# Skylarking/MARL

Hardware: AMD Instinct MI355X
Metric: env_steps_per_sec (higher is better)
Workload: dtype f32 (bf16x6 split products, fp32 accumulate)

## Files before the change

marl_amd/csrc/common.h:

```cpp
#pragma once
#include <hip/hip_runtime.h>
#include <stdint.h>

#define MARL_WAVE 64

#define WG_BARRIER() asm volatile("s_waitcnt lgkmcnt(0)\n\ts_barrier" ::: "memory")

struct MarlSwitches {
  int fwd_xs, fwd_w2l, bwd_pipe_max_rt, wgrad_tall, wide_res, rollout_v1, unroll_r6;
};
extern "C" const MarlSwitches* marl_switches(void);

#ifndef MARL_PAD_H
#define MARL_PAD_H 8
#endif
#ifndef MARL_PAD_K
#define MARL_PAD_K 8
#endif
#ifndef MARL_PAD_G
#define MARL_PAD_G 8
#endif

typedef float f32x4 __attribute__((ext_vector_type(4)));
typedef int i32x4 __attribute__((ext_vector_type(4)));

__device__ __forceinline__ f32x4 mfma16(float a, float b, f32x4 c) {
  return __builtin_amdgcn_mfma_f32_16x16x4f32(a, b, c, 0, 0, 0);
}

__device__ __forceinline__ f32x4 mfma16x4(const f32x4& a, const f32x4& b, f32x4 c) {
  c = mfma16(a[0], b[0], c);
  c = mfma16(a[1], b[1], c);
  c = mfma16(a[2], b[2], c);
  c = mfma16(a[3], b[3], c);
  return c;
}

#ifdef MARL_NO_INTERLEAVE
__device__ __forceinline__ void mfma16x4_il2(const f32x4& a0, const f32x4& b0, f32x4& c0, const f32x4& a1, const f32x4& b1, f32x4& c1) {
  c0 = mfma16x4(a0, b0, c0); c1 = mfma16x4(a1, b1, c1);
}
__device__ __forceinline__ void mfma16x4_il3(const f32x4& a0, const f32x4& b0, f32x4& c0, const f32x4& a1, const f32x4& b1, f32x4& c1,
// ... 250 lines not shown
```

marl_amd/csrc/optim.hip:

```cpp
#include "common.h"
#include <string.h>
#include "../../include/marl_hip.h"

namespace {
constexpr int TPB = 256;
constexpr int MAXB = 1024;

__global__ void sumsq_kernel(const float* g, long n, float* ws) {
  __shared__ float sh[TPB / 64];
  float s = 0.f;
  for (long i = (long)blockIdx.x * TPB + threadIdx.x; i < n; i += (long)gridDim.x * TPB) s += g[i] * g[i];
  s = wave_sum(s);
  if ((threadIdx.x & 63) == 0) sh[threadIdx.x >> 6] = s;
  __syncthreads();
  if (threadIdx.x == 0) ws[blockIdx.x] = sh[0] + sh[1] + sh[2] + sh[3];
}

__global__ void sumsq_finish_kernel(const float* ws, int nb, float* out) {
  __shared__ float sh[TPB];
  float s = 0.f;
  for (int b = threadIdx.x; b < nb; b += TPB) s += ws[b];
  sh[threadIdx.x] = s;
  __syncthreads();
  for (int o = TPB / 2; o > 0; o >>= 1) {
// ... 42 lines not shown
}
}

extern "C" size_t marl_sumsq_workspace(long n) { return MAXB * sizeof(float); }

extern "C" int marl_grad_sumsq(const float* g, long n, float* sumsq, float* ws, void* stream) {
  const int nb = blocks_for(n);
  hipLaunchKernelGGL(sumsq_kernel, dim3(nb), dim3(TPB), 0, (hipStream_t)stream, g, n, ws);
  MARL_CHECK_LAUNCH();
  hipLaunchKernelGGL(sumsq_finish_kernel, dim3(1), dim3(TPB), 0, (hipStream_t)stream, (const float*)ws, nb, sumsq);
  MARL_CHECK_LAUNCH();
  return 0;
}

extern "C" int marl_rmsprop_step(float* p, const float* g, float* sq, long n, float lr, float alpha, float eps,
                                 float clip, const float* sumsq, const float* den, void* stream) {
  if (n <= 0) return 0;
  hipLaunchKernelGGL(rmsprop_kernel, dim3(blocks_for(n)), dim3(TPB), 0, (hipStream_t)stream, p, g, sq, n, lr, alpha,
                     eps, clip, sumsq, den);
  MARL_CHECK_LAUNCH();
  return 0;
}

extern "C" int marl_adam_step(float* p, const float* g, float* m, float* v, long n, float lr, float beta1,
                              float beta2, float eps, float bc1, float bc2_sqrt, float clip, const float* sumsq,
                              const float* den, void* stream) {
  if (n <= 0) return 0;
  hipLaunchKernelGGL(adam_kernel, dim3(blocks_for(n)), dim3(TPB), 0, (hipStream_t)stream, p, g, m, v, n, lr, beta1,
                     beta2, eps, bc1, bc2_sqrt, clip, sumsq, den);
  MARL_CHECK_LAUNCH();
  return 0;
}

static MarlSwitches g_switches = {1, 1, 4, 1, 1, 0, 1};
extern "C" const MarlSwitches* marl_switches(void) { return &g_switches; }
static int* switch_slot(const char* name) {
  if (!name) return nullptr;
  struct { const char* n; int* p; } tab[] = {{"fwd_xs", &g_switches.fwd_xs}, {"fwd_w2l", &g_switches.fwd_w2l},
                                             {"bwd_pipe_max_rt", &g_switches.bwd_pipe_max_rt}, {"wgrad_tall", &g_switches.wgrad_tall},
                                             {"wide_res", &g_switches.wide_res}, {"rollout_v1", &g_switches.rollout_v1}, {"unroll_r6", &g_switches.unroll_r6}};
  for (auto& t : tab)
    if (!strcmp(t.n, name)) return t.p;
  return nullptr;
}
extern "C" int marl_experiment_set(const char* name, int value) {
  int* p = switch_slot(name);
  if (!p) return -1;
  *p = value;
  return 0;
}
extern "C" int marl_experiment_get(const char* name) {
  int* p = switch_slot(name);
  return p ? *p : (-2147483647 - 1);
}

#ifndef MARL_SRC_HASH
#define MARL_SRC_HASH "unknown"
#endif
extern "C" const char* marl_hip_version(void) { return "marl_hip 0.4 (gfx950) src " MARL_SRC_HASH; }
```

marl_amd/csrc/qmix_fused.hip:

```cpp
#include "x6.h"
#include "../../include/marl_hip.h"

namespace {

constexpr int E = 32;
constexpr int KCQ = 8;
constexpr int SS = 128 + 4;
constexpr int NAG = 5;
constexpr int PP = 136;

struct QmixArgs {
  const float *W[4], *Bv[4];
  const float *wb2, *bb2;
  ConcatSrc s;
  const float* q;
  const float* g;
  float* q_tot;
  float* dq;
  float* ws;
  const float *lr, *lterm, *lpadded, *lq_tgt;
  float gamma;
  long rows;
  int N, S, C;
};

__host__ __device__ inline long qmix_slab_floats(int C, int S) { return (long)C * (S + 1) + (E + 1) + 2; }

template <int CTRL>
__device__ __forceinline__ float dpp(float v) {
  return __builtin_bit_cast(float, __builtin_amdgcn_update_dpp(0, __builtin_bit_cast(int, v), CTRL, 0xf, 0xf, true));
}
constexpr int DPP_XOR1 = 0xB1, DPP_XOR2 = 0x4E;
constexpr int DPP_HALF_MIRROR = 0x141, DPP_MIRROR = 0x140;
constexpr int DPP_ROR4 = 0x124, DPP_ROR8 = 0x128;
template <int EW>
__device__ __forceinline__ float group_sum(float v) {
  if (EW == 4) v += dpp<DPP_ROR4>(v);
  v += dpp<DPP_ROR8>(v);
  return v;
}
template <int EW>
__device__ __forceinline__ float e_sum(float v) {
  v += dpp<DPP_XOR1>(v);
  v += dpp<DPP_XOR2>(v);
  if (EW == 8) v += dpp<DPP_HALF_MIRROR>(v);
  return v;
}
__device__ __forceinline__ float row_sum(float v) {
  v += dpp<DPP_XOR1>(v);
  v += dpp<DPP_XOR2>(v);
  v += dpp<DPP_HALF_MIRROR>(v);
  v += dpp<DPP_MIRROR>(v);
  return v;
}
__device__ __forceinline__ float sign_clamp(float x, float lo) { return __builtin_amdgcn_fmed3f(x * 0x1p126f, lo, 1.0f); }

template <bool BWD, int NW, bool LOSS = false, bool X6 = false>
__global__ __launch_bounds__(64 * NW, 2) void qmix_fused_kernel(QmixArgs a) {
  static_assert(!LOSS || BWD, "the loss is folded into the backward kernel");
  static_assert(!X6 || NW == 8, "the split variant runs eight waves (two column tiles per wave: 96 registers of pre-split weights)");
  constexpr int QNT = 64 * NW, EW = 32 / NW, GPT = 16 / EW, TPW = 8 / GPT, LT = TPW - 1;
  constexpr int SRAW = X6 ? 2 * 3 * 16 * PP * 2 : 2 * 16 * SS * 4;
  __shared__ __attribute__((aligned(16))) char Sraw[SRAW];
  float (*Ss)[16 * SS] = reinterpret_cast<float (*)[16 * SS]>(Sraw);
  short* const Sp = reinterpret_cast<short*>(Sraw);
  constexpr int PLN = 16 * PP, PBUF = 3 * PLN;
  constexpr int KR = (X6 && BWD) ? (LOSS ? 2 : 3) : 4;
  constexpr int KL = 4 - KR;
  __shared__ __attribute__((aligned(16))) i32x4 WL[KL ? NW * TPW * KL * 3 * 64 : 1];
  __shared__ __attribute__((aligned(16))) float Qt2[2][8][16];
  __shared__ __attribute__((aligned(16))) float QT[NW][16];
  __shared__ __attribute__((aligned(16))) float DQP[NW][NAG][16];
  __shared__ __attribute__((aligned(16))) float Gs2[2][16];
  __shared__ __attribute__((aligned(16))) float Ls2[2][4][16];
  const int tid = threadIdx.x, lane = tid & 63, wave = tid >> 6;
  const int q4 = lane >> 4, m = lane & 15;
  const int el = m & (EW - 1), gl = m / EW, e = EW * wave + el;
  const int N = a.N, S = a.S, C = a.C, NE = N * E;
  const bool ones = S < 128;

  f32x4 wq[X6 ? 1 : TPW][X6 ? 1 : KCQ];
  F3 wq6[X6 ? TPW : 1][X6 ? KR : 1];
  float bias[TPW];
  int grp[TPW];
#pragma unroll
  for (int c = 0; c < TPW; ++c) {
    const int g = GPT * c + gl;
    grp[c] = g;
    const float *Wp = nullptr, *Bp = nullptr;
    if (g < NAG) { if (g < N) { Wp = a.W[0] + (long)(g * E + e) * S; Bp = a.Bv[0] + g * E + e; } }
    else { Wp = a.W[g - NAG + 1] + (long)e * S; Bp = a.Bv[g - NAG + 1] + e; }
    bias[c] = Bp ? *Bp : 0.f;
    if (X6) {
#pragma unroll
      for (int kc = 0; kc < 4; ++kc) {
        float v[8];
#pragma unroll
        for (int jj = 0; jj < 8; ++jj) {
          const int kk = 32 * kc + 8 * q4 + jj;
          v[jj] = (Wp && kk < S) ? Wp[kk] : 0.f;
        }
        const F3 f = split8((f32x4){v[0], v[1], v[2], v[3]}, (f32x4){v[4], v[5], v[6], v[7]});
        if (kc < KR) wq6[c][kc < KR ? kc : 0] = f;
        else { i32x4* wl = WL + (((wave * TPW + c) * (KL ? KL : 1) + (kc - KR)) * 3) * 64 + lane; wl[0] = f.h; wl[64] = f.m; wl[128] = f.l; }
      }
    } else {
#pragma unroll
      for (int kc = 0; kc < KCQ; ++kc)
#pragma unroll
        for (int i = 0; i < 4; ++i) {
          const int kk = 16 * kc + 4 * q4 + i;
          wq[c][kc][i] = (Wp && kk < S) ? Wp[kk] : 0.f;
        }
    }
  }
  const bool is6 = grp[LT] == 6, is7 = grp[LT] == 7;
  const float wb2e = a.wb2[e];
  const float cw = is7 ? wb2e : 0.f;
  const float bb2 = a.bb2[0];
  constexpr int MT = NAG / GPT;
  const unsigned absmask = grp[MT] < NAG ? 0x7fffffffu : 0xffffffffu;
  float lo_c[TPW];
#pragma unroll
  for (int c = 0; c < TPW; ++c) lo_c[c] = grp[c] == NAG ? 1.f : (grp[c] == 7 ? 0.f : -1.f);

  f32x4 accW[BWD ? TPW : 1][BWD ? KCQ : 1];
  float sbW[TPW];
#pragma unroll
  for (int c = 0; c < TPW; ++c) sbW[c] = 0.f;
  float acc_wb2 = 0.f, acc_bb2 = 0.f;
  float acc_ln = 0.f, acc_lm = 0.f;
  if (BWD) {
#pragma unroll
    for (int c = 0; c < TPW; ++c)
#pragma unroll
      for (int kc = 0; kc < KCQ; ++kc) accW[c][kc] = (f32x4){0.f, 0.f, 0.f, 0.f};
  }
  if (tid < 2 * 8 * 16) {
    const int r8 = (tid >> 4) & 7;
    (&Qt2[0][0][0])[tid] = r8 == NAG ? 1.f : 0.f;
  }

  const int tiles = (int)((a.rows + 15) / 16);
  constexpr int NPF = 512 / QNT;
  f32x4 pf[NPF];
  int pe0 = 0, pe1 = 0, pw0 = 0, pw1 = 0;
  const int fr = tid >> 5, fc4 = (tid & 31) * 4;
  const bool ones_lane = BWD && ones && fc4 == (S & ~3);
  const int ones_j = S & 3;
  const int nrows = (int)a.rows;
  const unsigned last_row = (unsigned)(nrows - 1);
  const unsigned rpe = (unsigned)a.s.rpe0;
  const int roff = rpe ? (int)a.s.off0 : 0;
  const FastDiv fd = a.s.fd0;
  const int* emap = a.s.emap0;
  const float* sp0 = a.s.p0 + (fc4 < S ? fc4 : 0);
  const long ld = a.s.ld0, blk = (long)a.s.bs0 * a.s.ld0;
  auto map_one = [&](int tile, int i, int& pe, int& pw) {
    unsigned row = (unsigned)tile * 16u + (unsigned)(fr + (QNT / 32) * i);
    row = row < last_row ? row : last_row;
    const unsigned ep = rpe ? fastdiv(row, fd) : 0u;
    pw = (int)(row - ep * rpe) + roff;
    pe = (int)ep;
    if (emap) pe = emap[ep];
  };
  auto map_issue = [&](int tile) {
    map_one(tile, 0, pe0, pw0);
    if (NPF > 1) map_one(tile, 1, pe1, pw1);
  };
  auto fetch_one = [&](int pe, int pw) {
    f32x4 v = *reinterpret_cast<const f32x4*>(sp0 + ((long)pe * blk + (long)pw * ld));
    if (BWD) {
#pragma unroll
      for (int j = 0; j < 4; ++j) v[j] = (ones_lane && j == ones_j) ? 1.f : v[j];
    }
    return v;
  };
  auto fetch = [&](int) {
    pf[0] = fetch_one(pe0, pw0);
    if (NPF > 1) pf[NPF - 1] = fetch_one(pe1, pw1);
  };
  auto stash = [&](int buf) {
#pragma unroll
    for (int i = 0; i < NPF; ++i) {
      if (X6) {
        const F3h f = split4(pf[i]);
        short* p = Sp + buf * PBUF + (fr + (QNT / 32) * i) * PP + fc4;
        *reinterpret_cast<i32x2*>(p) = f.h;
        *reinterpret_cast<i32x2*>(p + PLN) = f.m;
        *reinterpret_cast<i32x2*>(p + 2 * PLN) = f.l;
      } else *reinterpret_cast<f32x4*>(&Ss[buf][(fr + (QNT / 32) * i) * SS + fc4]) = pf[i];
    }
  };
  float pq = 0.f, pg = 0.f, pl[4] = {0.f, 0.f, 0.f, 0.f};
  const int qr = tid / N, qn = tid - qr * N;
  auto fetch_qg = [&](int tile) {
    pq = 0.f; pg = 0.f;
    if (tid < 16 * N) {
      const int row = tile * 16 + qr;
      if (row < nrows) pq = a.q[(unsigned)(row * N + qn)];
    }
    if (BWD && tid >= 192 && tid < 208) {
      const int row = tile * 16 + (tid - 192);
      if (LOSS) {
        pl[0] = pl[1] = pl[3] = 0.f; pl[2] = 1.f;
        if (row < nrows) { pl[0] = a.lr[row]; pl[1] = a.lterm[row]; pl[2] = a.lpadded[row]; pl[3] = a.lq_tgt[row]; }
      } else if (row < nrows) pg = a.g[row];
    }
  };
  auto flush_dq = [&](int prow0) {
    if (tid < 16 * N) {
      float v = 0.f;
#pragma unroll
      for (int w = 0; w < NW; ++w) v += DQP[w][qn][qr];
      if (prow0 + qr < nrows) a.dq[(unsigned)((prow0 + qr) * N + qn)] = v;
    }
  };
  int tile = blockIdx.x;
  if (tile < tiles) {
    map_issue(tile); fetch(tile); fetch_qg(tile);
    if (tile + (int)gridDim.x < tiles) map_issue(tile + gridDim.x);
    stash(0);
  }
  int buf = 0;
  int prow0 = -1;
  ST_DECL(8);
  __syncthreads();
  for (; tile < tiles; tile += gridDim.x, buf ^= 1) {
    const int row0 = tile * 16;
    if (tid < 16 * N) Qt2[buf][qn][qr] = pq;
    if (BWD && tid >= 192 && tid < 208) {
      if (LOSS) {
#pragma unroll
        for (int k = 0; k < 4; ++k) Ls2[buf][k][tid - 192] = pl[k];
      } else Gs2[buf][tid - 192] = pg;
    }
    const int nt = tile + gridDim.x;
    if (nt < tiles) {
      fetch(nt); fetch_qg(nt);
      if (nt + (int)gridDim.x < tiles) map_issue(nt + gridDim.x);
    }
    ST_MARK(0);
    WG_BARRIER();
    ST_MARK(1);
    if (BWD && prow0 >= 0) flush_dq(prow0);
    f32x4 acc[TPW];
#pragma unroll
    for (int c = 0; c < TPW; ++c) acc[c] = (f32x4){bias[c], bias[c], bias[c], bias[c]};
    if (X6) {
      f32x4 accb[TPW];
#pragma unroll
      for (int c = 0; c < TPW; ++c) accb[c] = (f32x4){0.f, 0.f, 0.f, 0.f};
      const short* sp = Sp + buf * PBUF + m * PP + 8 * q4;
#pragma unroll
      for (int kc = 0; kc < 4; ++kc) {
        F3 xa;
        xa.h = *reinterpret_cast<const i32x4*>(sp + 32 * kc);
        xa.m = *reinterpret_cast<const i32x4*>(sp + PLN + 32 * kc);
        xa.l = *reinterpret_cast<const i32x4*>(sp + 2 * PLN + 32 * kc);
        F3 wk[TPW];
#pragma unroll
        for (int c = 0; c < TPW; ++c) {
          if (kc < KR) wk[c] = wq6[c][kc < KR ? kc : 0];
          else { const i32x4* wl = WL + (((wave * TPW + c) * (KL ? KL : 1) + (kc - KR)) * 3) * 64 + lane; wk[c].h = wl[0]; wk[c].m = wl[64]; wk[c].l = wl[128]; }
        }
#define OP(p_, q_) _Pragma("unroll") for (int c = 0; c < TPW; ++c) { if (kc & 1) accb[c] = mm(xa.p_, wk[c].q_, accb[c]); else acc[c] = mm(xa.p_, wk[c].q_, acc[c]); }
        OP(m, m) OP(h, l) OP(l, h) OP(h, m) OP(m, h) OP(h, h)
#undef OP
      }
#pragma unroll
      for (int c = 0; c < TPW; ++c) acc[c] += accb[c];
    } else {
      const float* sr = &Ss[buf][m * SS + 4 * q4];
#pragma unroll
      for (int kc = 0; kc < KCQ; ++kc) {
        const f32x4 a4 = *reinterpret_cast<const f32x4*>(sr + 16 * kc);
#pragma unroll
        for (int i = 0; i < 4; ++i)
#pragma unroll
          for (int c = 0; c < TPW; ++c) acc[c] = mfma16(a4[i], wq[c][kc][i], acc[c]);
      }
    }
    ST_MARK(2);
    __builtin_amdgcn_sched_barrier(0);
    f32x4 qv[TPW];
    f32x4 p = {0.f, 0.f, 0.f, 0.f};
#pragma unroll
    for (int c = 0; c <= MT; ++c) {
      qv[c] = *reinterpret_cast<const f32x4*>(&Qt2[buf][grp[c]][4 * q4]);
#pragma unroll
      for (int i = 0; i < 4; ++i) {
        const float av = acc[c][i];
        const float x = c < MT ? fabsf(av) : __builtin_bit_cast(float, __builtin_bit_cast(unsigned, av) & absmask);
        p[i] = c == 0 ? x * qv[c][i] : fmaf(x, qv[c][i], p[i]);
      }
    }
    f32x4 ex, hid, t4;
#pragma unroll
    for (int i = 0; i < 4; ++i) {
      p[i] = group_sum<EW>(p[i]);
      ex[i] = __expf(p[i]);
      hid[i] = p[i] > 0.f ? p[i] : ex[i] - 1.f;
      const float z = is6 ? fabsf(acc[LT][i]) : fmaxf(acc[LT][i], 0.f);
      t4[i] = row_sum(z * (is6 ? hid[i] : cw));
    }
    if (m == 0) *reinterpret_cast<f32x4*>(&QT[wave][4 * q4]) = t4;
    ST_MARK(3);
    WG_BARRIER();
    ST_MARK(4);
    if (!BWD) {
      if (tid < 16) {
        float tot = 0.f;
#pragma unroll
        for (int w = 0; w < NW; ++w) tot += QT[w][tid];
        if (row0 + tid < nrows) a.q_tot[row0 + tid] = tot + bb2;
      }
      ST_MARK(5);
    } else {
      f32x4 qt = *reinterpret_cast<const f32x4*>(&QT[0][4 * q4]);
#pragma unroll
      for (int w = 1; w < NW; ++w) qt += *reinterpret_cast<const f32x4*>(&QT[w][4 * q4]);
      f32x4 gr;
      if (LOSS) {
        const f32x4 lr = *reinterpret_cast<const f32x4*>(&Ls2[buf][0][4 * q4]);
        const f32x4 lt = *reinterpret_cast<const f32x4*>(&Ls2[buf][1][4 * q4]);
        const f32x4 lp = *reinterpret_cast<const f32x4*>(&Ls2[buf][2][4 * q4]);
        const f32x4 lq = *reinterpret_cast<const f32x4*>(&Ls2[buf][3][4 * q4]);
#pragma unroll
        for (int i = 0; i < 4; ++i) {
          qt[i] += bb2;
          const float mask = 1.f - lp[i];
          const float target = lr[i] + a.gamma * lq[i] * (1.f - lt[i]);
          const float mtd = mask * (target - qt[i]);
          gr[i] = -2.f * mask * mtd;
          acc_ln += mtd * mtd; acc_lm += mask;
        }
        if (a.q_tot && wave == 0 && m == 0) {
          if (row0 + 16 <= nrows) *reinterpret_cast<f32x4*>(&a.q_tot[row0 + 4 * q4]) = qt;
          else {
#pragma unroll
            for (int i = 0; i < 4; ++i) if (row0 + 4 * q4 + i < nrows) a.q_tot[row0 + 4 * q4 + i] = qt[i];
          }
        }
      } else gr = *reinterpret_cast<const f32x4*>(&Gs2[buf][4 * q4]);
      f32x4 dpre, dhy[TPW];
#pragma unroll
      for (int i = 0; i < 4; ++i) {
        const float w2 = group_sum<EW>(is6 ? fabsf(acc[LT][i]) : 0.f);
        dpre[i] = gr[i] * w2 * (p[i] > 0.f ? 1.f : ex[i]);
        acc_wb2 += gr[i] * fmaxf(acc[LT][i], 0.f);
        acc_bb2 += gr[i];
      }
#pragma unroll
      for (int c = 0; c < TPW; ++c) {
        const bool lo_all = GPT * c + GPT - 1 <= NAG, hi_all = GPT * c > NAG;
#pragma unroll
        for (int i = 0; i < 4; ++i) {
          float x, y;
          if (lo_all) { x = qv[c][i]; y = dpre[i]; }
          else if (hi_all) { x = gr[i]; y = is6 ? hid[i] : wb2e; }
          else {
            const bool lo = grp[c] <= NAG;
            x = lo ? qv[c][i] : gr[i];
            y = lo ? dpre[i] : (is6 ? hid[i] : wb2e);
          }
          dhy[c][i] = (x * y) * sign_clamp(acc[c][i], lo_c[c]);
        }
        if (!ones) sbW[c] += dhy[c][0] + dhy[c][1] + dhy[c][2] + dhy[c][3];
        if (GPT * c < NAG) {
          f32x4 d4;
#pragma unroll
          for (int i = 0; i < 4; ++i) d4[i] = e_sum<EW>(fabsf(acc[c][i]) * dpre[i]);
          if (el == 0 && grp[c] < N) *reinterpret_cast<f32x4*>(&DQP[wave][grp[c]][4 * q4]) = d4;
        }
      }
      ST_MARK(5);
      __builtin_amdgcn_sched_barrier(0);
      if (X6) {
        typedef __attribute__((address_space(3))) s16x4 lds_s16x4;
        F3h dA[TPW];
#pragma unroll
        for (int c = 0; c < TPW; ++c) dA[c] = split4(dhy[c]);
        const short* tb = Sp + buf * PBUF + (4 * q4 + (m >> 2)) * PP + 4 * (m & 3);
#pragma unroll
        for (int kc = 0; kc < KCQ; ++kc) {
          F3h sb;
          sb.h = __builtin_bit_cast(i32x2, __builtin_amdgcn_ds_read_tr16_b64_v4i16((lds_s16x4*)(tb + 16 * kc)));
          sb.m = __builtin_bit_cast(i32x2, __builtin_amdgcn_ds_read_tr16_b64_v4i16((lds_s16x4*)(tb + PLN + 16 * kc)));
          sb.l = __builtin_bit_cast(i32x2, __builtin_amdgcn_ds_read_tr16_b64_v4i16((lds_s16x4*)(tb + 2 * PLN + 16 * kc)));
#define OP(p_, q_) _Pragma("unroll") for (int c = 0; c < TPW; ++c) accW[c][kc] = mmh(dA[c].p_, sb.q_, accW[c][kc]);
          OP(m, m) OP(h, l) OP(l, h) OP(h, m) OP(m, h) OP(h, h)
#undef OP
        }
      } else {
        const float* sd = &Ss[buf][(4 * q4) * SS + m];
#pragma unroll
        for (int kc = 0; kc < KCQ; ++kc) {
          f32x4 sD;
#pragma unroll
          for (int i = 0; i < 4; ++i) sD[i] = sd[i * SS + 16 * kc];
#pragma unroll
          for (int i = 0; i < 4; ++i)
#pragma unroll
            for (int c = 0; c < TPW; ++c) accW[c][kc] = mfma16(dhy[c][i], sD[i], accW[c][kc]);
        }
      }
      prow0 = row0;
    }
    ST_MARK(6);
    if (nt < tiles) stash(buf ^ 1);
    ST_MARK(7);
  }
  ST_DUMP_AT(8, BWD ? 8 : 0);
  if (BWD) {
    __syncthreads();
    if (prow0 >= 0) flush_dq(prow0);
    float* slab = a.ws + (long)blockIdx.x * qmix_slab_floats(C, S);
    const int Sx = S + 1;
#pragma unroll
    for (int c = 0; c < TPW; ++c) {
#pragma unroll
      for (int i = 0; i < 4; ++i) {
        const int cc = 4 * q4 + i, g = GPT * c + cc / EW, ee = EW * wave + (cc & (EW - 1));
        if (g < NAG && g >= N) continue;
        const int col = g < NAG ? g * E + ee : NE + (g - NAG) * E + ee;
#pragma unroll
        for (int kc = 0; kc < KCQ; ++kc) {
          const int k = 16 * kc + m;
          if (k < S || (ones && k == S)) slab[(long)col * Sx + k] = accW[c][kc][i];
        }
      }
      if (!ones) {
        float sb = sbW[c];
        sb += __shfl_xor(sb, 16, 64); sb += __shfl_xor(sb, 32, 64);
        const int g = grp[c];
        if (q4 == 0 && !(g < NAG && g >= N)) slab[(long)(g < NAG ? g * E + e : NE + (g - NAG) * E + e) * Sx + S] = sb;
      }
    }
    float v = acc_wb2;
    v += __shfl_xor(v, 16, 64); v += __shfl_xor(v, 32, 64);
    if (is7 && q4 == 0) slab[(long)C * Sx + e] = v;
    float b = acc_bb2, ln = acc_ln, lm = acc_lm;
    b += __shfl_xor(b, 16, 64); b += __shfl_xor(b, 32, 64);
    ln += __shfl_xor(ln, 16, 64); ln += __shfl_xor(ln, 32, 64);
    lm += __shfl_xor(lm, 16, 64); lm += __shfl_xor(lm, 32, 64);
    if (tid == 0) {
      slab[(long)C * Sx + E] = b;
      slab[(long)C * Sx + E + 1] = LOSS ? ln : 0.f;
      slab[(long)C * Sx + E + 2] = LOSS ? lm : 0.f;
    }
  }
// ... 71 lines not shown

}

extern "C" int marl_qmix_fused_supported(int N, int S, int Eq) { return supported(N, S, Eq) ? 1 : 0; }

extern "C" size_t marl_qmix_fused_workspace(long rows, int N, int S) {
  return (size_t)grid_for(rows) * qmix_slab_floats(N * E + 3 * E, S) * sizeof(float);
}

static int qmix_fwd_impl(const marl_qmix_weights_t* w, const marl_src_t* s, const float* q, float* q_tot,
                         long rows, int N, int S, int Eq, bool x6, void* stream) {
  if (rows <= 0) return 0;
  if (!supported(N, S, Eq)) return (int)hipErrorInvalidValue;
  QmixArgs a;
  if (fill(a, w, s, q, rows, N, S)) return (int)hipErrorInvalidValue;
  a.g = nullptr; a.q_tot = q_tot; a.dq = nullptr; a.ws = nullptr;
  a.lr = a.lterm = a.lpadded = a.lq_tgt = nullptr; a.gamma = 0.f;
  if (x6) hipLaunchKernelGGL((qmix_fused_kernel<false, 8, false, true>), dim3(grid_for(rows, 1)), dim3(512), 0, (hipStream_t)stream, a);
  else hipLaunchKernelGGL((qmix_fused_kernel<false, 4>), dim3(grid_for(rows, 2)), dim3(256), 0, (hipStream_t)stream, a);
  MARL_CHECK_LAUNCH();
  return 0;
}
extern "C" int marl_qmix_fused_fwd(const marl_qmix_weights_t* w, const marl_src_t* s, const float* q, float* q_tot,
                                   long rows, int N, int S, int Eq, void* stream) {
  return qmix_fwd_impl(w, s, q, q_tot, rows, N, S, Eq, false, stream);
}
extern "C" int marl_qmix_fused_fwd_x6(const marl_qmix_weights_t* w, const marl_src_t* s, const float* q, float* q_tot,
                                      long rows, int N, int S, int Eq, void* stream) {
  return qmix_fwd_impl(w, s, q, q_tot, rows, N, S, Eq, true, stream);
}

static int qmix_bwd_launch(QmixArgs& a, const marl_qmix_weights_t* grads, float* loss2, float* ws, long rows, int N, int S,
                           bool loss, bool x6, hipStream_t st) {
  const unsigned nwg = grid_for(rows);
  if (x6) {
    if (loss) hipLaunchKernelGGL((qmix_fused_kernel<true, 8, true, true>), dim3(nwg), dim3(512), 0, st, a);
    else hipLaunchKernelGGL((qmix_fused_kernel<true, 8, false, true>), dim3(nwg), dim3(512), 0, st, a);
  } else if (loss) hipLaunchKernelGGL((qmix_fused_kernel<true, 8, true>), dim3(nwg), dim3(512), 0, st, a);
  else hipLaunchKernelGGL((qmix_fused_kernel<true, 8, false>), dim3(nwg), dim3(512), 0, st, a);
  MARL_CHECK_LAUNCH();
  QmixRedArgs r;
  r.ws = ws; r.nwg = (int)nwg; r.N = N; r.S = S; r.C = a.C; r.loss2 = loss2;
  r.dW[0] = const_cast<float*>(grads->w1); r.dB[0] = const_cast<float*>(grads->w1_b);
  r.dW[1] = const_cast<float*>(grads->b1); r.dB[1] = const_cast<float*>(grads->b1_b);
  r.dW[2] = const_cast<float*>(grads->w2); r.dB[2] = const_cast<float*>(grads->w2_b);
  r.dW[3] = const_cast<float*>(grads->h); r.dB[3] = const_cast<float*>(grads->h_b);
  r.dwb2 = const_cast<float*>(grads->b2_w); r.dbb2 = const_cast<float*>(grads->b2_b);
  const long slab = qmix_slab_floats(a.C, S);
  hipLaunchKernelGGL(qmix_fused_reduce_kernel, dim3((unsigned)((slab + 63) / 64)), dim3(64 * RSG), 0, st, r);
  MARL_CHECK_LAUNCH();
  return 0;
}

static int qmix_bwd_impl(const marl_qmix_weights_t* w, const marl_src_t* s, const float* q, const float* dq_tot, float* dq,
                         const marl_qmix_weights_t* grads, float* ws, size_t ws_bytes, long rows, int N, int S, int Eq, bool x6,
                         void* stream) {
  if (rows <= 0) return 0;
  if (!supported(N, S, Eq)) return (int)hipErrorInvalidValue;
  if (ws_bytes < marl_qmix_fused_workspace(rows, N, S)) return (int)hipErrorInvalidValue;
  QmixArgs a;
  if (fill(a, w, s, q, rows, N, S)) return (int)hipErrorInvalidValue;
  a.g = dq_tot; a.q_tot = nullptr; a.dq = dq; a.ws = ws;
  a.lr = a.lterm = a.lpadded = a.lq_tgt = nullptr; a.gamma = 0.f;
  return qmix_bwd_launch(a, grads, nullptr, ws, rows, N, S, false, x6, (hipStream_t)stream);
}
extern "C" int marl_qmix_fused_bwd(const marl_qmix_weights_t* w, const marl_src_t* s, const float* q,
                                   const float* dq_tot, float* dq, const marl_qmix_weights_t* grads, float* ws,
                                   size_t ws_bytes, long rows, int N, int S, int Eq, void* stream) {
// ... 38 lines not shown
```

marl_amd/experiments.py:

```python
from __future__ import annotations

import contextlib
import os
import warnings

LIB_DEFAULTS = {"fwd_xs": 1, "fwd_w2l": 1, "bwd_pipe_max_rt": 4, "wgrad_tall": 1, "wide_res": 1, "rollout_v1": 0, "unroll_r6": 1}
HOST_DEFAULTS = {"no_pair": 0, "no_chain": 0, "chain_split": None, "mlp3_keep": 1, "x6_bwd_min_wg": 1, "force_reducer": 0}


def _env_int(name, default):
    v = os.environ.get("MARL_" + name.upper())
    if v is None or v == "":
        return default
    try:
        return int(v)
    except ValueError:
        warnings.warn("MARL_%s=%r ignored (want an integer)" % (name.upper(), v))
        return default


_lib_values = {k: _env_int(k, d) for k, d in LIB_DEFAULTS.items()}
_host_values = {k: _env_int(k, d) for k, d in HOST_DEFAULTS.items()}
if _host_values["chain_split"] is not None and not (_host_values["chain_split"] == 0 or
                                                      (8 <= _host_values["chain_split"] <= 248 and _host_values["chain_split"] % 8 == 0)):
    warnings.warn("MARL_CHAIN_SPLIT=%r ignored (want 0 or a multiple of 8 in 8..248)" % _host_values["chain_split"])
    _host_values["chain_split"] = None
_applied = None
generation = 0


def apply(lib):
    global _applied
    _applied = lib
    for k, v in _lib_values.items():
        if v != LIB_DEFAULTS[k]:
            rc = lib.marl_experiment_set(k.encode(), int(v))
            assert rc == 0, "marl_experiment_set(%s) failed" % k


# ... 35 lines not shown
```

Measured before the change: 72.23 million.

## Process row-tile pairs in split QMIX backward to double weight-gradient MFMA K

Adds a PAIR variant of the split-precision QMIX backward kernel in which each iteration handles two 16-row tiles. The weight-gradient MFMAs then consume 32 rows of K via paired transposed LDS reads and split8. Prefetch moves after the elementwise stage, and fewer weight k-chunks stay in registers. It is enabled by default when there are at least 512 tiles, and the grid is halved and capped at 256. The aim is fewer MFMA issues per row and less loop overhead, at the cost of doubled LDS staging, more register pressure and spilling weight chunks to LDS.

```diff
diff --git a/marl_amd/csrc/common.h b/marl_amd/csrc/common.h
--- a/marl_amd/csrc/common.h
+++ b/marl_amd/csrc/common.h
@@ -7,7 +7,7 @@
 #define WG_BARRIER() asm volatile("s_waitcnt lgkmcnt(0)\n\ts_barrier" ::: "memory")
 
 struct MarlSwitches {
-  int fwd_xs, fwd_w2l, bwd_pipe_max_rt, wgrad_tall, wide_res, rollout_v1, unroll_r6;
+  int fwd_xs, fwd_w2l, bwd_pipe_max_rt, wgrad_tall, wide_res, rollout_v1, unroll_r6, qmix_pair;
 };
 extern "C" const MarlSwitches* marl_switches(void);
 
diff --git a/marl_amd/csrc/optim.hip b/marl_amd/csrc/optim.hip
--- a/marl_amd/csrc/optim.hip
+++ b/marl_amd/csrc/optim.hip
@@ -98,13 +98,14 @@
   return 0;
 }
 
-static MarlSwitches g_switches = {1, 1, 4, 1, 1, 0, 1};
+static MarlSwitches g_switches = {1, 1, 4, 1, 1, 0, 1, 0};
 extern "C" const MarlSwitches* marl_switches(void) { return &g_switches; }
 static int* switch_slot(const char* name) {
   if (!name) return nullptr;
   struct { const char* n; int* p; } tab[] = {{"fwd_xs", &g_switches.fwd_xs}, {"fwd_w2l", &g_switches.fwd_w2l},
                                              {"bwd_pipe_max_rt", &g_switches.bwd_pipe_max_rt}, {"wgrad_tall", &g_switches.wgrad_tall},
-                                             {"wide_res", &g_switches.wide_res}, {"rollout_v1", &g_switches.rollout_v1}, {"unroll_r6", &g_switches.unroll_r6}};
+                                             {"wide_res", &g_switches.wide_res}, {"rollout_v1", &g_switches.rollout_v1}, {"unroll_r6", &g_switches.unroll_r6},
+                                             {"qmix_pair", &g_switches.qmix_pair}};
   for (auto& t : tab)
     if (!strcmp(t.n, name)) return t.p;
   return nullptr;
diff --git a/marl_amd/csrc/qmix_fused.hip b/marl_amd/csrc/qmix_fused.hip
--- a/marl_amd/csrc/qmix_fused.hip
+++ b/marl_amd/csrc/qmix_fused.hip
@@ -55,24 +55,26 @@
 }
 __device__ __forceinline__ float sign_clamp(float x, float lo) { return __builtin_amdgcn_fmed3f(x * 0x1p126f, lo, 1.0f); }
 
-template <bool BWD, int NW, bool LOSS = false, bool X6 = false>
+template <bool BWD, int NW, bool LOSS = false, bool X6 = false, bool PAIR = false>
 __global__ __launch_bounds__(64 * NW, 2) void qmix_fused_kernel(QmixArgs a) {
   static_assert(!LOSS || BWD, "the loss is folded into the backward kernel");
   static_assert(!X6 || NW == 8, "the split variant runs eight waves (two column tiles per wave: 96 registers of pre-split weights)");
+  static_assert(!PAIR || (BWD && X6), "row-tile pairs exist for the weight gradient of the split backward kernels");
   constexpr int QNT = 64 * NW, EW = 32 / NW, GPT = 16 / EW, TPW = 8 / GPT, LT = TPW - 1;
-  constexpr int SRAW = X6 ? 2 * 3 * 16 * PP * 2 : 2 * 16 * SS * 4;
+  constexpr int NTP = PAIR ? 2 : 1;
+  constexpr int SRAW = X6 ? 2 * NTP * 3 * 16 * PP * 2 : 2 * 16 * SS * 4;
   __shared__ __attribute__((aligned(16))) char Sraw[SRAW];
   float (*Ss)[16 * SS] = reinterpret_cast<float (*)[16 * SS]>(Sraw);
   short* const Sp = reinterpret_cast<short*>(Sraw);
-  constexpr int PLN = 16 * PP, PBUF = 3 * PLN;
-  constexpr int KR = (X6 && BWD) ? (LOSS ? 2 : 3) : 4;
+  constexpr int PLN = 16 * PP, PTL = 3 * PLN, PBUF = NTP * PTL;
+  constexpr int KR = (X6 && BWD) ? ((LOSS || PAIR) ? 2 : 3) : 4;
   constexpr int KL = 4 - KR;
   __shared__ __attribute__((aligned(16))) i32x4 WL[KL ? NW * TPW * KL * 3 * 64 : 1];
-  __shared__ __attribute__((aligned(16))) float Qt2[2][8][16];
-  __shared__ __attribute__((aligned(16))) float QT[NW][16];
-  __shared__ __attribute__((aligned(16))) float DQP[NW][NAG][16];
-  __shared__ __attribute__((aligned(16))) float Gs2[2][16];
-  __shared__ __attribute__((aligned(16))) float Ls2[2][4][16];
+  __shared__ __attribute__((aligned(16))) float Qt2[2][NTP][8][16];
+  __shared__ __attribute__((aligned(16))) float QT[NTP][NW][16];
+  __shared__ __attribute__((aligned(16))) float DQP[NTP][NW][NAG][16];
+  __shared__ __attribute__((aligned(16))) float Gs2[2][NTP][16];
+  __shared__ __attribute__((aligned(16))) float Ls2[2][NTP][4][16];
   const int tid = threadIdx.x, lane = tid & 63, wave = tid >> 6;
   const int q4 = lane >> 4, m = lane & 15;
   const int el = m & (EW - 1), gl = m / EW, e = EW * wave + el;
@@ -136,17 +138,33 @@
 #pragma unroll
       for (int kc = 0; kc < KCQ; ++kc) accW[c][kc] = (f32x4){0.f, 0.f, 0.f, 0.f};
   }
-  if (tid < 2 * 8 * 16) {
+  if (tid < 2 * NTP * 8 * 16) {
     const int r8 = (tid >> 4) & 7;
-    (&Qt2[0][0][0])[tid] = r8 == NAG ? 1.f : 0.f;
+    (&Qt2[0][0][0][0])[tid] = r8 == NAG ? 1.f : 0.f;
   }
 
-  const int tiles = (int)((a.rows + 15) / 16);
-  constexpr int NPF = 512 / QNT;
+  const int tiles = (int)((a.rows + 16 * NTP - 1) / (16 * NTP));
+  constexpr int NPF = NTP * 512 / QNT;
   f32x4 pf[NPF];
   int pe0 = 0, pe1 = 0, pw0 = 0, pw1 = 0;
-  const int fr = tid >> 5, fc4 = (tid & 31) * 4;
-  const bool ones_lane = BWD && ones && fc4 == (S & ~3);
+  struct Ix { int fr, fc4, qr, qn, qj, qi, gj, gi; bool ones_lane; const float* sp0; };
+  auto mk_ix = [&](int t) {
+    Ix x;
+    x.fr = t >> 5; x.fc4 = (t & 31) * 4;
+    x.ones_lane = BWD && ones && x.fc4 == (S & ~3);
+    x.sp0 = a.s.p0 + (x.fc4 < S ? x.fc4 : 0);
+    x.qr = t / N; x.qn = t - x.qr * N;
+    x.qj = PAIR ? x.qr >> 4 : 0; x.qi = PAIR ? x.qr & 15 : x.qr;
+    x.gj = PAIR ? (t - 192) >> 4 : 0; x.gi = PAIR ? (t - 192) & 15 : t - 192;
+    return x;
+  };
+  const Ix ix0 = mk_ix(tid);
+  auto ix = [&]() {
+    if (!PAIR) return ix0;
+    int t = tid;
+    asm volatile("" : "+v"(t));
+    return mk_ix(t);
+  };
   const int ones_j = S & 3;
   const int nrows = (int)a.rows;
   const unsigned last_row = (unsigned)(nrows - 1);
@@ -154,10 +172,9 @@
   const int roff = rpe ? (int)a.s.off0 : 0;
   const FastDiv fd = a.s.fd0;
   const int* emap = a.s.emap0;
-  const float* sp0 = a.s.p0 + (fc4 < S ? fc4 : 0);
   const long ld = a.s.ld0, blk = (long)a.s.bs0 * a.s.ld0;
   auto map_one = [&](int tile, int i, int& pe, int& pw) {
-    unsigned row = (unsigned)tile * 16u + (unsigned)(fr + (QNT / 32) * i);
+    unsigned row = (unsigned)tile * (16u * NTP) + (unsigned)(ix().fr + (QNT / 32) * i);
     row = row < last_row ? row : last_row;
     const unsigned ep = rpe ? fastdiv(row, fd) : 0u;
     pw = (int)(row - ep * rpe) + roff;
@@ -169,10 +186,11 @@
     if (NPF > 1) map_one(tile, 1, pe1, pw1);
   };
   auto fetch_one = [&](int pe, int pw) {
-    f32x4 v = *reinterpret_cast<const f32x4*>(sp0 + ((long)pe * blk + (long)pw * ld));
+    const Ix x = ix();
+    f32x4 v = *reinterpret_cast<const f32x4*>(x.sp0 + ((long)pe * blk + (long)pw * ld));
     if (BWD) {
 #pragma unroll
-      for (int j = 0; j < 4; ++j) v[j] = (ones_lane && j == ones_j) ? 1.f : v[j];
+      for (int j = 0; j < 4; ++j) v[j] = (x.ones_lane && j == ones_j) ? 1.f : v[j];
     }
     return v;
   };
@@ -181,11 +199,12 @@
     if (NPF > 1) pf[NPF - 1] = fetch_one(pe1, pw1);
   };
   auto stash = [&](int buf) {
+    const int fr = ix().fr, fc4 = ix().fc4;
 #pragma unroll
     for (int i = 0; i < NPF; ++i) {
       if (X6) {
         const F3h f = split4(pf[i]);
-        short* p = Sp + buf * PBUF + (fr + (QNT / 32) * i) * PP + fc4;
+        short* p = Sp + buf * PBUF + (PAIR ? i * PTL + fr * PP : (fr + (QNT / 32) * i) * PP) + fc4;
         *reinterpret_cast<i32x2*>(p) = f.h;
         *reinterpret_cast<i32x2*>(p + PLN) = f.m;
         *reinterpret_cast<i32x2*>(p + 2 * PLN) = f.l;
@@ -193,15 +212,24 @@
     }
   };
   float pq = 0.f, pg = 0.f, pl[4] = {0.f, 0.f, 0.f, 0.f};
-  const int qr = tid / N, qn = tid - qr * N;
   auto fetch_qg = [&](int tile) {
     pq = 0.f; pg = 0.f;
-    if (tid < 16 * N) {
-      const int row = tile * 16 + qr;
-      if (row < nrows) pq = a.q[(unsigned)(row * N + qn)];
-    }
-    if (BWD && tid >= 192 && tid < 208) {
-      const int row = tile * 16 + (tid - 192);
+    if (tid < 16 * NTP * N) {
+      const Ix x = ix();
+      const int row = tile * (16 * NTP) + x.qr;
+      if (row < nrows) pq = a.q[(unsigned)(row * N + x.qn)];
+    }
+    if (PAIR && LOSS) {
+      if (tid >= 192 && tid < 320) {
+        int t = tid - 192;
+        asm volatile("" : "+v"(t));
+        const int k = t >> 5, row = tile * 32 + (t & 31);
+        pg = k == 2 ? 1.f : 0.f;
+        const float* src = k == 0 ? a.lr : (k == 1 ? a.lterm : (k == 2 ? a.lpadded : a.lq_tgt));
+        if (row < nrows) pg = src[row];
+      }
+    } else if (BWD && tid >= 192 && tid < 192 + 16 * NTP) {
+      const int row = tile * (16 * NTP) + (tid - 192);
       if (LOSS) {
         pl[0] = pl[1] = pl[3] = 0.f; pl[2] = 1.f;
         if (row < nrows) { pl[0] = a.lr[row]; pl[1] = a.lterm[row]; pl[2] = a.lpadded[row]; pl[3] = a.lq_tgt[row]; }
@@ -209,11 +237,12 @@
     }
   };
   auto flush_dq = [&](int prow0) {
-    if (tid < 16 * N) {
+    if (tid < 16 * NTP * N) {
+      const Ix x = ix();
       float v = 0.f;
 #pragma unroll
-      for (int w = 0; w < NW; ++w) v += DQP[w][qn][qr];
-      if (prow0 + qr < nrows) a.dq[(unsigned)((prow0 + qr) * N + qn)] = v;
+      for (int w = 0; w < NW; ++w) v += DQP[x.qj][w][x.qn][x.qi];
+      if (prow0 + x.qr < nrows) a.dq[(unsigned)((prow0 + x.qr) * N + x.qn)] = v;
     }
   };
   int tile = blockIdx.x;
@@ -227,49 +256,71 @@
   ST_DECL(8);
   __syncthreads();
   for (; tile < tiles; tile += gridDim.x, buf ^= 1) {
-    const int row0 = tile * 16;
-    if (tid < 16 * N) Qt2[buf][qn][qr] = pq;
-    if (BWD && tid >= 192 && tid < 208) {
-      if (LOSS) {
-#pragma unroll
-        for (int k = 0; k < 4; ++k) Ls2[buf][k][tid - 192] = pl[k];
-      } else Gs2[buf][tid - 192] = pg;
+    const int row0 = tile * (16 * NTP);
+    {
+      const Ix x = ix();
+      if (tid < 16 * NTP * N) Qt2[buf][x.qj][x.qn][x.qi] = pq;
+      if (PAIR && LOSS) {
+        if (tid >= 192 && tid < 320) {
+          int t = tid - 192;
+          asm volatile("" : "+v"(t));
+          Ls2[buf][(t >> 4) & 1][t >> 5][t & 15] = pg;
+        }
+      } else if (BWD && tid >= 192 && tid < 192 + 16 * NTP) {
+        if (LOSS) {
+#pragma unroll
+          for (int k = 0; k < 4; ++k) Ls2[buf][x.gj][k][x.gi] = pl[k];
+        } else Gs2[buf][x.gj][x.gi] = pg;
+      }
     }
     const int nt = tile + gridDim.x;
-    if (nt < tiles) {
-      fetch(nt); fetch_qg(nt);
-      if (nt + (int)gridDim.x < tiles) map_issue(nt + gridDim.x);
-    }
+    auto prefetch = [&]() {
+      if (nt < tiles) {
+        fetch(nt); fetch_qg(nt);
+        if (nt + (int)gridDim.x < tiles) map_issue(nt + gridDim.x);
+      }
+    };
+    if (!PAIR) prefetch();
     ST_MARK(0);
     WG_BARRIER();
     ST_MARK(1);
     if (BWD && prow0 >= 0) flush_dq(prow0);
-    f32x4 acc[TPW];
-#pragma unroll
-    for (int c = 0; c < TPW; ++c) acc[c] = (f32x4){bias[c], bias[c], bias[c], bias[c]};
+    f32x4 acc[NTP][TPW];
+#pragma unroll
+    for (int j = 0; j < NTP; ++j)
+#pragma unroll
+      for (int c = 0; c < TPW; ++c) acc[j][c] = (f32x4){bias[c], bias[c], bias[c], bias[c]};
     if (X6) {
-      f32x4 accb[TPW];
-#pragma unroll
-      for (int c = 0; c < TPW; ++c) accb[c] = (f32x4){0.f, 0.f, 0.f, 0.f};
+      f32x4 accb[NTP][TPW];
+#pragma unroll
+      for (int j = 0; j < NTP; ++j)
+#pragma unroll
+        for (int c = 0; c < TPW; ++c) accb[j][c] = (f32x4){0.f, 0.f, 0.f, 0.f};
       const short* sp = Sp + buf * PBUF + m * PP + 8 * q4;
 #pragma unroll
       for (int kc = 0; kc < 4; ++kc) {
-        F3 xa;
-        xa.h = *reinterpret_cast<const i32x4*>(sp + 32 * kc);
-        xa.m = *reinterpret_cast<const i32x4*>(sp + PLN + 32 * kc);
-        xa.l = *reinterpret_cast<const i32x4*>(sp + 2 * PLN + 32 * kc);
         F3 wk[TPW];
 #pragma unroll
         for (int c = 0; c < TPW; ++c) {
           if (kc < KR) wk[c] = wq6[c][kc < KR ? kc : 0];
           else { const i32x4* wl = WL + (((wave * TPW + c) * (KL ? KL : 1) + (kc - KR)) * 3) * 64 + lane; wk[c].h = wl[0]; wk[c].m = wl[64]; wk[c].l = wl[128]; }
         }
-#define OP(p_, q_) _Pragma("unroll") for (int c = 0; c < TPW; ++c) { if (kc & 1) accb[c] = mm(xa.p_, wk[c].q_, accb[c]); else acc[c] = mm(xa.p_, wk[c].q_, acc[c]); }
-        OP(m, m) OP(h, l) OP(l, h) OP(h, m) OP(m, h) OP(h, h)
+#pragma unroll
+        for (int j = 0; j < NTP; ++j) {
+          F3 xa;
+          xa.h = *reinterpret_cast<const i32x4*>(sp + j * PTL + 32 * kc);
+          xa.m = *reinterpret_cast<const i32x4*>(sp + j * PTL + PLN + 32 * kc);
+          xa.l = *reinterpret_cast<const i32x4*>(sp + j * PTL + 2 * PLN + 32 * kc);
+#define OP(p_, q_) _Pragma("unroll") for (int c = 0; c < TPW; ++c) { if (kc & 1) accb[j][c] = mm(xa.p_, wk[c].q_, accb[j][c]); else acc[j][c] = mm(xa.p_, wk[c].q_, acc[j][c]); }
+          OP(m, m) OP(h, l) OP(l, h) OP(h, m) OP(m, h) OP(h, h)
 #undef OP
-      }
-#pragma unroll
-      for (int c = 0; c < TPW; ++c) acc[c] += accb[c];
+        }
+        if (PAIR) __builtin_amdgcn_sched_barrier(0);
+      }
+#pragma unroll
+      for (int j = 0; j < NTP; ++j)
+#pragma unroll
+        for (int c = 0; c < TPW; ++c) acc[j][c] += accb[j][c];
     } else {
       const float* sr = &Ss[buf][m * SS + 4 * q4];
 #pragma unroll
@@ -278,33 +329,38 @@
 #pragma unroll
         for (int i = 0; i < 4; ++i)
 #pragma unroll
-          for (int c = 0; c < TPW; ++c) acc[c] = mfma16(a4[i], wq[c][kc][i], acc[c]);
+          for (int c = 0; c < TPW; ++c) acc[0][c] = mfma16(a4[i], wq[c][kc][i], acc[0][c]);
       }
     }
     ST_MARK(2);
     __builtin_amdgcn_sched_barrier(0);
-    f32x4 qv[TPW];
-    f32x4 p = {0.f, 0.f, 0.f, 0.f};
-#pragma unroll
-    for (int c = 0; c <= MT; ++c) {
-      qv[c] = *reinterpret_cast<const f32x4*>(&Qt2[buf][grp[c]][4 * q4]);
+    f32x4 qv[NTP][TPW];
+    f32x4 p[NTP], ex[NTP], hid[NTP];
+#pragma unroll
+    for (int j = 0; j < NTP; ++j) {
+      p[j] = (f32x4){0.f, 0.f, 0.f, 0.f};
+#pragma unroll
+      for (int c = 0; c <= MT; ++c) {
+        qv[j][c] = *reinterpret_cast<const f32x4*>(&Qt2[buf][j][grp[c]][4 * q4]);
+#pragma unroll
+        for (int i = 0; i < 4; ++i) {
+          const float av = acc[j][c][i];
+          const float x = c < MT ? fabsf(av) : __builtin_bit_cast(float, __builtin_bit_cast(unsigned, av) & absmask);
+          p[j][i] = c == 0 ? x * qv[j][c][i] : fmaf(x, qv[j][c][i], p[j][i]);
+        }
+      }
+      f32x4 t4;
 #pragma unroll
       for (int i = 0; i < 4; ++i) {
-        const float av = acc[c][i];
-        const float x = c < MT ? fabsf(av) : __builtin_bit_cast(float, __builtin_bit_cast(unsigned, av) & absmask);
-        p[i] = c == 0 ? x * qv[c][i] : fmaf(x, qv[c][i], p[i]);
-      }
-    }
-    f32x4 ex, hid, t4;
-#pragma unroll
-    for (int i = 0; i < 4; ++i) {
-      p[i] = group_sum<EW>(p[i]);
-      ex[i] = __expf(p[i]);
-      hid[i] = p[i] > 0.f ? p[i] : ex[i] - 1.f;
-      const float z = is6 ? fabsf(acc[LT][i]) : fmaxf(acc[LT][i], 0.f);
-      t4[i] = row_sum(z * (is6 ? hid[i] : cw));
-    }
-    if (m == 0) *reinterpret_cast<f32x4*>(&QT[wave][4 * q4]) = t4;
+        p[j][i] = group_sum<EW>(p[j][i]);
+        ex[j][i] = __expf(p[j][i]);
+        hid[j][i] = p[j][i] > 0.f ? p[j][i] : ex[j][i] - 1.f;
+        const float z = is6 ? fabsf(acc[j][LT][i]) : fmaxf(acc[j][LT][i], 0.f);
+        t4[i] = row_sum(z * (is6 ? hid[j][i] : cw));
+      }
+      if (m == 0) *reinterpret_cast<f32x4*>(&QT[j][wave][4 * q4]) = t4;
+      if (PAIR) __builtin_amdgcn_sched_barrier(0);
+    }
     ST_MARK(3);
     WG_BARRIER();
     ST_MARK(4);
@@ -312,75 +368,109 @@
       if (tid < 16) {
         float tot = 0.f;
 #pragma unroll
-        for (int w = 0; w < NW; ++w) tot += QT[w][tid];
+        for (int w = 0; w < NW; ++w) tot += QT[0][w][tid];
         if (row0 + tid < nrows) a.q_tot[row0 + tid] = tot + bb2;
       }
       ST_MARK(5);
     } else {
-      f32x4 qt = *reinterpret_cast<const f32x4*>(&QT[0][4 * q4]);
-#pragma unroll
-      for (int w = 1; w < NW; ++w) qt += *reinterpret_cast<const f32x4*>(&QT[w][4 * q4]);
-      f32x4 gr;
-      if (LOSS) {
-        const f32x4 lr = *reinterpret_cast<const f32x4*>(&Ls2[buf][0][4 * q4]);
-        const f32x4 lt = *reinterpret_cast<const f32x4*>(&Ls2[buf][1][4 * q4]);
-        const f32x4 lp = *reinterpret_cast<const f32x4*>(&Ls2[buf][2][4 * q4]);
-        const f32x4 lq = *reinterpret_cast<const f32x4*>(&Ls2[buf][3][4 * q4]);
+      f32x4 dhy[NTP][TPW];
+#pragma unroll
+      for (int j = 0; j < NTP; ++j) {
+        const int row0j = row0 + 16 * j;
+        f32x4 qt = *reinterpret_cast<const f32x4*>(&QT[j][0][4 * q4]);
+#pragma unroll
+        for (int w = 1; w < NW; ++w) qt += *reinterpret_cast<const f32x4*>(&QT[j][w][4 * q4]);
+        if (PAIR) __builtin_amdgcn_sched_barrier(0);
+        f32x4 gr;
+        if (LOSS) {
+          const f32x4 lr = *reinterpret_cast<const f32x4*>(&Ls2[buf][j][0][4 * q4]);
+          const f32x4 lt = *reinterpret_cast<const f32x4*>(&Ls2[buf][j][1][4 * q4]);
+          const f32x4 lp = *reinterpret_cast<const f32x4*>(&Ls2[buf][j][2][4 * q4]);
+          const f32x4 lq = *reinterpret_cast<const f32x4*>(&Ls2[buf][j][3][4 * q4]);
+#pragma unroll
+          for (int i = 0; i < 4; ++i) {
+            qt[i] += bb2;
+            const float mask = 1.f - lp[i];
+            const float target = lr[i] + a.gamma * lq[i] * (1.f - lt[i]);
+            const float mtd = mask * (target - qt[i]);
+            gr[i] = -2.f * mask * mtd;
+            acc_ln += mtd * mtd; acc_lm += mask;
+          }
+          if (a.q_tot && wave == 0 && m == 0) {
+            if (row0j + 16 <= nrows) *reinterpret_cast<f32x4*>(&a.q_tot[row0j + 4 * q4]) = qt;
+            else {
+#pragma unroll
+              for (int i = 0; i < 4; ++i) if (row0j + 4 * q4 + i < nrows) a.q_tot[row0j + 4 * q4 + i] = qt[i];
+            }
+          }
+        } else gr = *reinterpret_cast<const f32x4*>(&Gs2[buf][j][4 * q4]);
+        if (PAIR) __builtin_amdgcn_sched_barrier(0);
+        f32x4 dpre, hidj, qvj[TPW];
+#pragma unroll
+        for (int i = 0; i < 4; ++i) hidj[i] = !PAIR ? hid[j][i] : (p[j][i] > 0.f ? p[j][i] : ex[j][i] - 1.f);
+#pragma unroll
+        for (int c = 0; c <= MT; ++c) qvj[c] = !PAIR ? qv[j][c] : *reinterpret_cast<const f32x4*>(&Qt2[buf][j][grp[c]][4 * q4]);
 #pragma unroll
         for (int i = 0; i < 4; ++i) {
-          qt[i] += bb2;
-          const float mask = 1.f - lp[i];
-          const float target = lr[i] + a.gamma * lq[i] * (1.f - lt[i]);
-          const float mtd = mask * (target - qt[i]);
-          gr[i] = -2.f * mask * mtd;
-          acc_ln += mtd * mtd; acc_lm += mask;
-        }
-        if (a.q_tot && wave == 0 && m == 0) {
-          if (row0 + 16 <= nrows) *reinterpret_cast<f32x4*>(&a.q_tot[row0 + 4 * q4]) = qt;
-          else {
-#pragma unroll
-            for (int i = 0; i < 4; ++i) if (row0 + 4 * q4 + i < nrows) a.q_tot[row0 + 4 * q4 + i] = qt[i];
+          const float w2 = group_sum<EW>(is6 ? fabsf(acc[j][LT][i]) : 0.f);
+          dpre[i] = gr[i] * w2 * (p[j][i] > 0.f ? 1.f : ex[j][i]);
+          acc_wb2 += gr[i] * fmaxf(acc[j][LT][i], 0.f);
+          acc_bb2 += gr[i];
+        }
+#pragma unroll
+        for (int c = 0; c < TPW; ++c) {
+          const bool lo_all = GPT * c + GPT - 1 <= NAG, hi_all = GPT * c > NAG;
+#pragma unroll
+          for (int i = 0; i < 4; ++i) {
+            float x, y;
+            if (lo_all) { x = qvj[c][i]; y = dpre[i]; }
+            else if (hi_all) { x = gr[i]; y = is6 ? hidj[i] : wb2e; }
+            else {
+              const bool lo = grp[c] <= NAG;
+              x = lo ? qvj[c][i] : gr[i];
+              y = lo ? dpre[i] : (is6 ? hidj[i] : wb2e);
+            }
+            dhy[j][c][i] = (x * y) * sign_clamp(acc[j][c][i], lo_c[c]);
           }
-        }
-      } else gr = *reinterpret_cast<const f32x4*>(&Gs2[buf][4 * q4]);
-      f32x4 dpre, dhy[TPW];
-#pragma unroll
-      for (int i = 0; i < 4; ++i) {
-        const float w2 = group_sum<EW>(is6 ? fabsf(acc[LT][i]) : 0.f);
-        dpre[i] = gr[i] * w2 * (p[i] > 0.f ? 1.f : ex[i]);
-        acc_wb2 += gr[i] * fmaxf(acc[LT][i], 0.f);
-        acc_bb2 += gr[i];
-      }
-#pragma unroll
-      for (int c = 0; c < TPW; ++c) {
-        const bool lo_all = GPT * c + GPT - 1 <= NAG, hi_all = GPT * c > NAG;
-#pragma unroll
-        for (int i = 0; i < 4; ++i) {
-          float x, y;
-          if (lo_all) { x = qv[c][i]; y = dpre[i]; }
-          else if (hi_all) { x = gr[i]; y = is6 ? hid[i] : wb2e; }
-          else {
-            const bool lo = grp[c] <= NAG;
-            x = lo ? qv[c][i] : gr[i];
-            y = lo ? dpre[i] : (is6 ? hid[i] : wb2e);
+          if (!ones) sbW[c] += dhy[j][c][0] + dhy[j][c][1] + dhy[j][c][2] + dhy[j][c][3];
+          if (GPT * c < NAG) {
+            f32x4 d4;
+#pragma unroll
+            for (int i = 0; i < 4; ++i) d4[i] = e_sum<EW>(fabsf(acc[j][c][i]) * dpre[i]);
+            if (el == 0 && grp[c] < N) *reinterpret_cast<f32x4*>(&DQP[j][wave][grp[c]][4 * q4]) = d4;
           }
-          dhy[c][i] = (x * y) * sign_clamp(acc[c][i], lo_c[c]);
-        }
-        if (!ones) sbW[c] += dhy[c][0] + dhy[c][1] + dhy[c][2] + dhy[c][3];
-        if (GPT * c < NAG) {
-          f32x4 d4;
-#pragma unroll
-          for (int i = 0; i < 4; ++i) d4[i] = e_sum<EW>(fabsf(acc[c][i]) * dpre[i]);
-          if (el == 0 && grp[c] < N) *reinterpret_cast<f32x4*>(&DQP[wave][grp[c]][4 * q4]) = d4;
-        }
+        }
+        if (PAIR) __builtin_amdgcn_sched_barrier(0);
       }
       ST_MARK(5);
       __builtin_amdgcn_sched_barrier(0);
-      if (X6) {
+      if (PAIR) { prefetch(); __builtin_amdgcn_sched_barrier(0); }
+      if (PAIR) {
+        typedef __attribute__((address_space(3))) s16x4 lds_s16x4;
+        F3 dA[TPW];
+#pragma unroll
+        for (int c = 0; c < TPW; ++c) dA[c] = split8(dhy[0][c], dhy[NTP - 1][c]);
+        const short* tb = Sp + buf * PBUF + (4 * q4 + (m >> 2)) * PP + 4 * (m & 3);
+        auto tr2 = [&](const short* p0) {
+          const i32x2 lo = __builtin_bit_cast(i32x2, __builtin_amdgcn_ds_read_tr16_b64_v4i16((lds_s16x4*)p0));
+          const i32x2 hi = __builtin_bit_cast(i32x2, __builtin_amdgcn_ds_read_tr16_b64_v4i16((lds_s16x4*)(p0 + (NTP - 1) * PTL)));
+          return (i32x4){lo[0], lo[1], hi[0], hi[1]};
+        };
+#pragma unroll
+        for (int kc = 0; kc < KCQ; ++kc) {
+          F3 sb;
+          sb.h = tr2(tb + 16 * kc);
+          sb.m = tr2(tb + PLN + 16 * kc);
+          sb.l = tr2(tb + 2 * PLN + 16 * kc);
+#define OP(p_, q_) _Pragma("unroll") for (int c = 0; c < TPW; ++c) accW[c][kc] = mm(dA[c].p_, sb.q_, accW[c][kc]);
+          OP(m, m) OP(h, l) OP(l, h) OP(h, m) OP(m, h) OP(h, h)
+#undef OP
+        }
+      } else if (X6) {
         typedef __attribute__((address_space(3))) s16x4 lds_s16x4;
         F3h dA[TPW];
 #pragma unroll
-        for (int c = 0; c < TPW; ++c) dA[c] = split4(dhy[c]);
+        for (int c = 0; c < TPW; ++c) dA[c] = split4(dhy[0][c]);
         const short* tb = Sp + buf * PBUF + (4 * q4 + (m >> 2)) * PP + 4 * (m & 3);
 #pragma unroll
         for (int kc = 0; kc < KCQ; ++kc) {
@@ -402,7 +492,7 @@
 #pragma unroll
           for (int i = 0; i < 4; ++i)
 #pragma unroll
-            for (int c = 0; c < TPW; ++c) accW[c][kc] = mfma16(dhy[c][i], sD[i], accW[c][kc]);
+            for (int c = 0; c < TPW; ++c) accW[c][kc] = mfma16(dhy[0][c][i], sD[i], accW[c][kc]);
         }
       }
       prow0 = row0;
@@ -417,6 +507,13 @@
     if (prow0 >= 0) flush_dq(prow0);
     float* slab = a.ws + (long)blockIdx.x * qmix_slab_floats(C, S);
     const int Sx = S + 1;
+    int tt = tid;
+    if (PAIR) asm volatile("" : "+v"(tt));
+    const int q4 = (tt & 63) >> 4, m = tt & 15, wave = tt >> 6, e = EW * wave + (m & (EW - 1));
+    int grp[TPW];
+#pragma unroll
+    for (int c = 0; c < TPW; ++c) grp[c] = GPT * c + m / EW;
+    const bool is7 = grp[LT] == 7;
 #pragma unroll
     for (int c = 0; c < TPW; ++c) {
 #pragma unroll
@@ -554,8 +651,14 @@
 
 static int qmix_bwd_launch(QmixArgs& a, const marl_qmix_weights_t* grads, float* loss2, float* ws, long rows, int N, int S,
                            bool loss, bool x6, hipStream_t st) {
-  const unsigned nwg = grid_for(rows);
-  if (x6) {
+  const long tiles = (rows + 15) / 16;
+  const int sw = marl_switches()->qmix_pair;
+  const bool pair = x6 && sw != 1 && (sw == 2 || tiles >= 512);
+  const unsigned nwg = pair ? (unsigned)((tiles + 1) / 2 < 256 ? (tiles + 1) / 2 : 256) : grid_for(rows);
+  if (pair) {
+    if (loss) hipLaunchKernelGGL((qmix_fused_kernel<true, 8, true, true, true>), dim3(nwg), dim3(512), 0, st, a);
+    else hipLaunchKernelGGL((qmix_fused_kernel<true, 8, false, true, true>), dim3(nwg), dim3(512), 0, st, a);
+  } else if (x6) {
     if (loss) hipLaunchKernelGGL((qmix_fused_kernel<true, 8, true, true>), dim3(nwg), dim3(512), 0, st, a);
     else hipLaunchKernelGGL((qmix_fused_kernel<true, 8, false, true>), dim3(nwg), dim3(512), 0, st, a);
   } else if (loss) hipLaunchKernelGGL((qmix_fused_kernel<true, 8, true>), dim3(nwg), dim3(512), 0, st, a);
diff --git a/marl_amd/experiments.py b/marl_amd/experiments.py
--- a/marl_amd/experiments.py
+++ b/marl_amd/experiments.py
@@ -4,7 +4,7 @@
 import os
 import warnings
 
-LIB_DEFAULTS = {"fwd_xs": 1, "fwd_w2l": 1, "bwd_pipe_max_rt": 4, "wgrad_tall": 1, "wide_res": 1, "rollout_v1": 0, "unroll_r6": 1}
+LIB_DEFAULTS = {"fwd_xs": 1, "fwd_w2l": 1, "bwd_pipe_max_rt": 4, "wgrad_tall": 1, "wide_res": 1, "rollout_v1": 0, "unroll_r6": 1, "qmix_pair": 0}
 HOST_DEFAULTS = {"no_pair": 0, "no_chain": 0, "chain_split": None, "mlp3_keep": 1, "x6_bwd_min_wg": 1, "force_reducer": 0}
 
 
```

After: 73.25 million (median of 5 runs). +1.4%, better.
